# antarcticrainforest/seabreeze_param

Hardware: AMD Instinct MI355X
Metric: grid-points/sec for sea_breeze_diag on N2560x1920 global grid; achieved HBM GB/s (higher is better)
Workload: dtype f64; 1 GPU; seabreeze_diag generic flavour, N1280 (2560x1920) global grid, nz=56, fp64 (BASELINE.json configs[2]); stream=torch's current stream (torch and the library share one HIP runtime), plan_cache=stored, nx=2560, ny=1920, nz=56, search_halo=16, parallelism=latband1, variant=default, comm=none, multi_rank_rccl=unmeasured on hardware so far (one GPU per box in the build pool)

## Files before the change

include/seabreeze_hip.h:

```cpp
#ifndef SEABREEZE_HIP_H
#define SEABREEZE_HIP_H

#include <stddef.h>
#include <stdint.h>

#ifdef __cplusplus
extern "C" {
#endif

typedef struct sb_ctx sb_ctx;

typedef enum sb_status {
    SB_OK = 0,
    SB_ERR_ARG = 1,
    SB_ERR_HIP = 2,
    SB_ERR_NO_DEVICE = 3,
    SB_ERR_ALLOC = 4,
    SB_ERR_COMM = 5
} sb_status;

typedef enum sb_boundary {
    SB_BND_WRAPPER = 0,
    SB_BND_GLOBAL = 1,
    SB_BND_HALO = 2
} sb_boundary;

typedef struct sb_tunables {
    double target_plev_pa;
    double thresh_wind;
    double thresh_winddir;
    double thresh_windch;
    double thresh_thc;
    double target_time_s;
    double maxdist_km;
} sb_tunables;

int  sb_create(sb_ctx **ctx, int device);
int  sb_destroy(sb_ctx *ctx);
const char *sb_last_error(const sb_ctx *ctx);
const char *sb_version(void);
void sb_default_tunables(sb_tunables *t);
int  sb_set_search_radius_hint(sb_ctx *ctx, int radius);
int  sb_set_fold(sb_ctx *ctx, int on);
int  sb_set_plan_cache(sb_ctx *ctx, int on);
int  sb_set_wide_strip(sb_ctx *ctx, int on);
int  sb_set_band_order(sb_ctx *ctx, int contrast_first);
int  sb_set_workgroups(sb_ctx *ctx, int n);
int  sb_set_static_sigma(sb_ctx *ctx, int on);
int  sb_set_table_contrast(sb_ctx *ctx, int on);
int  sb_set_table_window_cache(sb_ctx *ctx, int on);
int  sb_table_cache_report(sb_ctx *ctx, long long rep[4]);
int  sb_last_step_report(sb_ctx *ctx, int report[4]);
int  sb_last_counters(sb_ctx *ctx, long long counters[4]);
int  sb_synchronize(sb_ctx *ctx);
int  sb_profile_begin(sb_ctx *ctx, int max_calls);
int  sb_profile_end(sb_ctx *ctx, double avg_ms[5], int *ncalls);

int sb_seabreeze_diag_f64(sb_ctx *ctx, double timestep_s, int timestep_number,
                          int nx, int ny, int nz, int halo, int bnd,
                          const double *p, const double *u, const double *v,
                          const double *theta, const double *mask, const double *z,
                          const double *sigma, double *windspeed, double *winddir,
                          double *thc, double *sb_con, const sb_tunables *tun);
int sb_seabreeze_diag_f32(sb_ctx *ctx, float timestep_s, int timestep_number,
                          int nx, int ny, int nz, int halo, int bnd,
                          const float *p, const float *u, const float *v,
                          const float *theta, const float *mask, const float *z,
                          const float *sigma, float *windspeed, float *winddir,
                          float *thc, float *sb_con, const sb_tunables *tun);
int sb_seabreeze_diag_f64_dev(sb_ctx *ctx, double timestep_s, int timestep_number,
                          int nx, int ny, int nz, int halo, int bnd,
                          const double *p, const double *u, const double *v,
                          const double *theta, const double *mask, const double *z,
                          const double *sigma, double *windspeed, double *winddir,
                          double *thc, double *sb_con, const sb_tunables *tun,
                          void *stream);
int sb_seabreeze_diag_f32_dev(sb_ctx *ctx, float timestep_s, int timestep_number,
                          int nx, int ny, int nz, int halo, int bnd,
                          const float *p, const float *u, const float *v,
                          const float *theta, const float *mask, const float *z,
                          const float *sigma, float *windspeed, float *winddir,
                          float *thc, float *sb_con, const sb_tunables *tun,
                          void *stream);

#define SB_UM_THETA_TO_T0 1
#define SB_UM_LEVEL_WALK  2
int sb_seabreeze_diag_um_f64(sb_ctx *ctx, double timestep_s, int timestep_number, int nx, int ny, int nz,
                             int halo_s, int halo_l, const double *p, const double *u, const double *v,
                             double *theta, const double *z, const double *sigma, const double *mask,
                             double *windspeed, double *winddir, double *thc, double *sb_con, int flags,
                             int *error);
int sb_seabreeze_diag_um_f32(sb_ctx *ctx, float timestep_s, int timestep_number, int nx, int ny, int nz,
                             int halo_s, int halo_l, const float *p, const float *u, const float *v,
                             float *theta, const float *z, const float *sigma, const float *mask,
                             float *windspeed, float *winddir, float *thc, float *sb_con, int flags,
                             int *error);
int sb_seabreeze_diag_um_f64_dev(sb_ctx *ctx, double timestep_s, int timestep_number, int nx, int ny, int nz,
                             int halo_s, int halo_l, const double *p, const double *u, const double *v,
                             double *theta, const double *z, const double *sigma, const double *mask,
// ... 176 lines not shown
```

seabreeze_param_amd/csrc/sb_capi.hip:

```cpp
#include "../../include/seabreeze_hip.h"
#include "sb_launch.hpp"

#include <dlfcn.h>
#include <rccl/rccl.h>

#include <algorithm>
#include <chrono>
#include <cmath>
#include <condition_variable>
#include <functional>
#include <mutex>
#include <thread>
#include <cstdio>
#include <cstdlib>
#include <cstring>
#include <string>
#include <vector>

namespace {

thread_local std::string g_err;

struct DevBuf {
    void *p = nullptr;
// ... 45 lines not shown
            }
        }
    }
    void loop() {
        unsigned long seen = 0;
        for (;;) {
            {
                std::unique_lock<std::mutex> lk(m_);
                cv_.wait(lk, [&] { return quit_ || epoch_ != seen; });
                if (quit_) return;
                seen = epoch_;
            }
            work();
        }
    }
    std::vector<std::thread> workers_;
    std::mutex m_;
    std::condition_variable cv_, done_cv_;
    const std::function<void(int)> *fn_ = nullptr;
    int next_ = 0, total_ = 0, done_ = 0;
    unsigned long epoch_ = 0;
    bool quit_ = false;
};

enum { SB_TICKET_WORDS = 2 };

struct DiagStream {
    bool active = false;
    HostPool *pool = nullptr;
    int nlons = 0, nlats = 0, esz = 0;
    DevBuf z, sd, cdist, ws, wd, thc, p1, theta, v, u, out;
    void *pin_in[2] = {nullptr, nullptr};
    void *pin_out[2] = {nullptr, nullptr};
    size_t pin_in_cap = 0, pin_out_cap = 0;
    hipEvent_t ev_in[2] = {nullptr, nullptr}, ev_out[2] = {nullptr, nullptr};
    long steps = 0;
    double host_copy_s = 0.0, enqueue_s = 0.0, wait_s = 0.0;
};

struct sb_ctx {
    int device = 0;
    hipStream_t stream = nullptr;
    std::string err;
    int radius_hint = 16;
    int ncu = 256;
    int ncu_dev = 256;
    int static_sigma = 0;
    bool stats_valid = false;
    int host_depth = 0;
    int no_fold = 0;
    int no_plan_cache = 0;
    int no_wide_strip = 0;
    int band_late_wind = 0;
    int table_contrast = 0;
    int table_cache = 0;
    SbTabCache tabc;
    bool tab_rep_reset = true;
    bool tab_last = false;
    long long tab_calls = 0;
    int tab_waves = 0;
    const void *stats_sigma = nullptr;
    int stats_dims[4] = {0, 0, 0, 0};
    int stats_ngathered = 0;
    int rep_launches = 0, rep_rccl = 0, rep_groups = 0, rep_copies = 0;
    DevBuf t0, bandbits, clsbits, tiles, vecs, nws, nwd, coastbits, tile_list, seg_list, stamps, jobcopy, plan;
    DevBuf umbits;
    DevBuf tabA, tabL, tabC, tabS;
    DevBuf tabW, tabRep;
    int plan_key[8] = {0, 0, 0, 0, 0, 0, 0, 0};
    const void *plan_bits = nullptr;
    int call_seq = 0, plan_use = 0;
    bool segs_built = false;
    int tiles_n = 0, tiles_strip = -1, flag_parity = 0;
    int *last_flags = nullptr;
    Moments *partials = nullptr;
    unsigned int *ticket = nullptr;
    void *stats = nullptr;
    int *counters = nullptr;
    int *seg_count = nullptr;
    std::vector<unsigned char> dist_key, dist_hv;
    SbDistTraits dist_traits;
    hipStream_t dist_upload_stream = nullptr;
    std::vector<DevBuf> stage;
    Geo last_g{};
    int last_tiles = 0;
    bool have_last = false;
    const Moments *gathered = nullptr;
    int ngathered = 0;
    std::vector<hipEvent_t> prof_ev;
    std::vector<unsigned> prof_mask;
    int prof_calls = 0, prof_max = 0;
    hipStream_t aux_stream = nullptr;
    hipEvent_t ev_fork = nullptr, ev_join = nullptr, ev_mom = nullptr;
    Moments *band_moments_out = nullptr;
    int band_geo = 0;
    DevBuf band_mom;
    void *rccl_lib = nullptr;
    void *comm = nullptr;
    int rank = 0, nranks = 1;
    DiagStream ds;
};

namespace {

int fail(sb_ctx *c, int code, const std::string &msg) {
    if (c) c->err = msg; else g_err = msg;
// ... 88 lines not shown
    const size_t nseg = (size_t)g.nyh * g.nw;
    const size_t seg_cap = (nseg + SB_SEG_PARTS - 1) / SB_SEG_PARTS;
    if ((rc = ensure(c, c->seg_list, seg_cap * SB_SEG_PARTS * sizeof(SbSegEntry)))) return rc;
    job.tile_list = (int *)c->tile_list.p;
    job.seg_list = (SbSegEntry *)c->seg_list.p;
    job.seg_count = c->seg_count;
    job.seg_cap = (int)seg_cap;
    job.t0_fly = (job.flavour == SB_FLAVOUR_GENERIC) ? 1 : 0;
    if (!job.t0_fly) {
        if ((rc = ensure(c, c->t0, ncell * sizeof(T)))) return rc;
        job.t0 = (T *)c->t0.p;
    }
    if ((rc = ensure(c, c->jobcopy, sizeof(DiagJob<double>)))) return rc;
    job.self = (DiagJob<T> *)c->jobcopy.p;
    const bool cache = c->table_cache != 0 && c->table_contrast != 0 && job.flavour == SB_FLAVOUR_GENERIC &&
                       (g.bnd == BND_GLOBAL || g.bnd == BND_HALO) && g.band == 0 && phases == 3 && c->gathered == nullptr;
    if (strip || cache) {
        const size_t need = 64 + (strip ? (size_t)c->ncu * SB_PLAN_STRIDE : (size_t)0);
        if (c->plan.cap < need) {
            if ((rc = ensure(c, c->plan, need))) return rc;
            HIPCHK(c, hipMemsetAsync(c->plan.p, 0, need, st));
            c->plan_bits = nullptr;
        }
        if (phases & 1) {
            if (c->call_seq == 0x7fffffff) {
                HIPCHK(c, hipMemsetAsync(c->plan.p, 0, need, st));
                c->call_seq = 0;
                c->plan_bits = nullptr;
            }
            ++c->call_seq;
            if (strip) {
                const int key[8] = {g.nx, g.ny, g.h, g.bnd, g.rows, c->ncu, tx, ty | (vb << 24)};
                c->plan_use = c->plan_bits == c->bandbits.p && std::memcmp(key, c->plan_key, sizeof(key)) == 0 ? 1 : 0;
                std::memcpy(c->plan_key, key, sizeof(key));
                c->plan_bits = c->bandbits.p;
            } else c->plan_bits = nullptr;
        }
        job.plan = (char *)c->plan.p + 64;
        job.plan_gen = (int *)c->plan.p;
        job.call_id = c->call_seq;
        job.plan_use = strip && !c->no_plan_cache ? c->plan_use : 0;
    } else if (phases & 1) c->plan_bits = nullptr;
#ifdef SB_STAMPS
    if ((rc = ensure(c, c->stamps, (size_t)4096 * SB_NSTAMP * sizeof(long long)))) return rc;
    job.stamps = (long long *)c->stamps.p;
#endif
    SbLaunchCtx lc{};
    if (phases == 3 && c->prof_calls < c->prof_max) {
        lc.prof_mask = &c->prof_mask[(size_t)c->prof_calls];
        lc.prof = &c->prof_ev[(size_t)SB_PROF_EVENTS * c->prof_calls++];
    }
    lc.stream = st; lc.partials = c->partials; lc.stats = c->stats;
    lc.gathered = c->gathered; lc.ngathered = c->ngathered; lc.ncu = c->ncu;
    lc.moments_out = (phases == 1) ? c->band_moments_out : nullptr;
    lc.moments_event = (phases == 1 && c->nranks > 1) ? c->ev_mom : nullptr;
    lc.stats_ticket = (int *)c->ticket + 1;
    in.phases = phases; in.t0_fly = job.t0_fly != 0; in.moments_out = lc.moments_out != nullptr;
    in.reuse_stats = reuse_stats<T>(c, job.sigma, g.nx, g.ny, g.h);
    in.plan_use = c->plan_use != 0; in.segs_built = c->segs_built;
    in.scan_wgs = sb_scan_workgroups((unsigned)g.nyh * (unsigned)g.nw, c->ncu);
    in.table = c->table_contrast != 0 && job.flavour == SB_FLAVOUR_GENERIC && (g.bnd == BND_GLOBAL || g.bnd == BND_HALO) && g.band == 0;
    const SbDiagPlan plan = sb_plan_diag(in);
    if (plan.table) {
        const size_t nsum = (size_t)((g.nyh + SB_TAB_RB - 1) / SB_TAB_RB) * g.nxh;
        if ((rc = ensure(c, c->tabA, ncell * sizeof(unsigned long long)))) return rc;
        if ((rc = ensure(c, c->tabL, ncell * sizeof(unsigned long long)))) return rc;
        if ((rc = ensure(c, c->tabC, ncell * sizeof(unsigned)))) return rc;
        if ((rc = ensure(c, c->tabS, nsum * (2 * sizeof(unsigned long long) + sizeof(unsigned))))) return rc;
        lc.tables.A = (unsigned long long *)c->tabA.p; lc.tables.L = (unsigned long long *)c->tabL.p; lc.tables.C = (unsigned *)c->tabC.p;
        lc.tables.SA = (unsigned long long *)c->tabS.p; lc.tables.SL = lc.tables.SA + nsum; lc.tables.SC = (unsigned *)(lc.tables.SL + nsum);
    }
    SbTabKey tkey{};
    if (plan.table && cache) {
        if ((rc = ensure(c, c->tabW, (size_t)g.nx * g.ny * sizeof(unsigned)))) return rc;
        if ((rc = ensure(c, c->tabRep, (SB_TAB_REP_HDR + (size_t)2 * SB_TAB_QUERY_WAVES_PER_CU * c->ncu_dev) * sizeof(unsigned)))) return rc;
        tkey = SbTabKey{g.nx, g.ny, g.h, g.bnd, g.rows, c->bandbits.p, c->clsbits.p, c->tabW.p, c->tabC.p};
        lc.tables.W = (unsigned *)c->tabW.p; lc.tables.rep = (unsigned *)c->tabRep.p;
        lc.tables.gen = job.plan_gen; lc.tables.call_id = job.call_id;
        lc.tables.force = sb_tab_cache_decide(c->tabc, tkey, job.call_id) != SB_TAB_STEADY ? 1 : 0;
        lc.tables.rep_reset = c->tab_rep_reset ? 1 : 0;
    }
    if (plan.wind_scratch) {
        if ((rc = ensure(c, c->nws, (size_t)g.nx * g.ny * sizeof(T)))) return rc;
        if ((rc = ensure(c, c->nwd, (size_t)g.nx * g.ny * sizeof(T)))) return rc;
        job.nws = (T *)c->nws.p; job.nwd = (T *)c->nwd.p;
    }
    if (phases == 3) c->rep_launches = c->rep_rccl = c->rep_groups = c->rep_copies = 0;
    {
        const hipError_t le = sb_launch_diag<T>(job, plan, lc);
        if (le != hipSuccess) {
            c->plan_bits = nullptr;
            c->segs_built = false;
            c->stats_valid = false;
            sb_tab_cache_launch_failed(c->tabc);
        }
        if (le == hipErrorInvalidValue) return fail(c, SB_ERR_ARG, "no contrast kernel instance for this halo / tile shape");
        if (le != hipSuccess) return hipfail(c, le, "sb_launch_diag");
    }
    c->rep_launches += plan.nsteps;
    if (lc.tables.W) {
        sb_tab_cache_filled(c->tabc, tkey, job.call_id);
        c->tab_rep_reset = false;
        c->tab_waves = SB_TAB_QUERY_WAVES_PER_CU * c->ncu;
        ++c->tab_calls;
    } else sb_tab_cache_other_call(c->tabc);
    c->tab_last = lc.tables.W != nullptr;
// ... 1264 lines not shown
    if (dptr) HIPCHK(c, hipFree(dptr));
    return SB_OK;
}
int sb_device_upload(sb_ctx *c, void *dst_dev, const void *src_host, size_t nbytes) {
    if (!c) return fail(nullptr, SB_ERR_ARG, "null context");
    if (!dst_dev || !src_host) return fail(c, SB_ERR_ARG, "null pointer");
    HIPCHK(c, hipMemcpyAsync(dst_dev, src_host, nbytes, hipMemcpyHostToDevice, c->stream));
    HIPCHK(c, hipStreamSynchronize(c->stream));
    return SB_OK;
}
int sb_device_download(sb_ctx *c, void *dst_host, const void *src_dev, size_t nbytes) {
    if (!c) return fail(nullptr, SB_ERR_ARG, "null context");
    if (!dst_host || !src_dev) return fail(c, SB_ERR_ARG, "null pointer");
    HIPCHK(c, hipMemcpyAsync(dst_host, src_dev, nbytes, hipMemcpyDeviceToHost, c->stream));
    HIPCHK(c, hipStreamSynchronize(c->stream));
    return SB_OK;
}

int sb_allgather_moments_dev(sb_ctx *c, const double *mine5, double *gathered, void *stream) {
    if (!c) return fail(nullptr, SB_ERR_ARG, "null context");
    if (!mine5 || !gathered) return fail(c, SB_ERR_ARG, "null pointer");
    hipStream_t st = stream ? (hipStream_t)stream : c->stream;
    if (c->nranks == 1) {
        HIPCHK(c, hipMemcpyAsync(gathered, mine5, 5 * sizeof(double), hipMemcpyDeviceToDevice, st));
        c->rep_copies += 1;
        return SB_OK;
    }
    NCCLCHK(c, g_rccl.AllGather(mine5, gathered, 5, ncclDouble, (ncclComm_t)c->comm, st));
    c->rep_rccl += 1;
    return SB_OK;
}

int sb_set_fold(sb_ctx *c, int on) {
    if (!c) return fail(nullptr, SB_ERR_ARG, "null context");
    c->no_fold = on ? 0 : 1;
    return SB_OK;
}

int sb_set_workgroups(sb_ctx *c, int n) {
    if (!c) return fail(nullptr, SB_ERR_ARG, "null context");
    if (n < 0 || n > c->ncu_dev) return fail(c, SB_ERR_ARG, "sb_set_workgroups: 0 (the default) or 1 .. the device's compute units");
    HIPCHK(c, hipDeviceSynchronize());
    c->ncu = n == 0 ? c->ncu_dev : n;
    c->plan_bits = nullptr;
    return SB_OK;
}

int sb_set_band_order(sb_ctx *c, int contrast_first) {
    if (!c) return fail(nullptr, SB_ERR_ARG, "null context");
    c->band_late_wind = contrast_first ? 1 : 0;
    return SB_OK;
}

int sb_set_plan_cache(sb_ctx *c, int on) {
    if (!c) return fail(nullptr, SB_ERR_ARG, "null context");
    c->no_plan_cache = on ? 0 : 1;
    return SB_OK;
}

int sb_set_wide_strip(sb_ctx *c, int on) {
    if (!c) return fail(nullptr, SB_ERR_ARG, "null context");
    c->no_wide_strip = on ? 0 : 1;
    c->plan_bits = nullptr;
    return SB_OK;
}

int sb_set_static_sigma(sb_ctx *c, int on) {
    if (!c) return fail(nullptr, SB_ERR_ARG, "null context");
    c->static_sigma = on ? 1 : 0;
    c->stats_valid = false;
    return SB_OK;
}

int sb_set_table_contrast(sb_ctx *c, int on) {
    if (!c) return fail(nullptr, SB_ERR_ARG, "null context");
    c->table_contrast = on ? 1 : 0;
    return SB_OK;
}

int sb_set_table_window_cache(sb_ctx *c, int on) {
    if (!c) return fail(nullptr, SB_ERR_ARG, "null context");
    c->table_cache = on ? 1 : 0;
    sb_tab_cache_toggled(c->tabc);
    if (on) { c->tab_rep_reset = true; c->tab_calls = 0; }
    return SB_OK;
}

int sb_table_cache_report(sb_ctx *c, long long rep[4]) {
    if (!c) return fail(nullptr, SB_ERR_ARG, "null context");
    if (!rep) return fail(c, SB_ERR_ARG, "null pointer");
    rep[0] = rep[1] = rep[2] = rep[3] = 0;
    if (c->tab_rep_reset || !c->tabRep.p) return SB_OK;
    HIPCHK(c, hipDeviceSynchronize());
    std::vector<unsigned> d(SB_TAB_REP_HDR + (size_t)2 * c->tab_waves);
    HIPCHK(c, hipMemcpy(d.data(), c->tabRep.p, d.size() * sizeof(unsigned), hipMemcpyDeviceToHost));
    if (c->tab_last)
        for (int w = 0; w < c->tab_waves; ++w) { rep[0] += d[SB_TAB_REP_HDR + 2 * w]; rep[1] += d[SB_TAB_REP_HDR + 2 * w + 1]; }
    rep[2] = d[0]; rep[3] = c->tab_calls;
    return SB_OK;
}

int sb_last_step_report(sb_ctx *c, int report[4]) {
    if (!c) return fail(nullptr, SB_ERR_ARG, "null context");
    if (!report) return fail(c, SB_ERR_ARG, "null pointer");
    report[0] = c->rep_launches; report[1] = c->rep_rccl; report[2] = c->rep_groups; report[3] = c->rep_copies;
    return SB_OK;
// ... 5 lines not shown
```

seabreeze_param_amd/csrc/sb_diag_kernels.hip:

```cpp
#include "sb_device.hpp"
#include "sb_launch.hpp"
#include "sb_scan_body.hpp"

#define STATS_NT SB_STATS_NT

__device__ __forceinline__ Moments moments_from_shifted(double c, double s1, double s2, double mn, double mx,
                                                         int cnt) {
    Moments acc = moments_empty();
    if (cnt > 0) {
        acc.n = (double)cnt;
        acc.mean = c + s1 / acc.n;
        acc.m2 = s2 - s1 * s1 / acc.n;
        acc.mn = mn;
        acc.mx = mx;
    }
    return acc;
}

__device__ __forceinline__ void store_partial(Moments acc, Moments *wpart, Moments *__restrict__ partials) {
    acc = block_merge(acc, wpart);
    if (threadIdx.x == 0) partials[blockIdx.x] = acc;
}

template <typename T>
__global__ __launch_bounds__(STATS_NT) void k_stats(const T *__restrict__ ary, int nx, int ny, int ld,
                                                    size_t off0, Moments *__restrict__ partials, int *__restrict__ ticket,
                                                    T *__restrict__ stats, Moments *__restrict__ moments_out) {
    const unsigned n = (unsigned)nx * (unsigned)ny;
    const unsigned stride = gridDim.x * STATS_NT;
    const bool flat = (ld == nx);
    const double c = (double)ary[off0];
    double s1 = 0.0, s2 = 0.0, mn = 1.0e308, mx = -1.0e308;
    int cnt = 0;
    for (unsigned base = blockIdx.x * STATS_NT + threadIdx.x; base < n; base += 8 * stride) {
        double x[8];
#pragma unroll
        for (int q = 0; q < 8; ++q) {
            const unsigned i = base + q * stride;
            x[q] = c;
            if (i < n) {
                const size_t idx = flat ? (size_t)i : (size_t)(i / (unsigned)nx) * ld + (i % (unsigned)nx);
                x[q] = (double)ary[off0 + idx];
            }
        }
#pragma unroll
        for (int q = 0; q < 8; ++q) {
            if (base + q * stride < n) {
                const double d = x[q] - c;
                s1 += d;
                s2 += d * d;
                mn = x[q] < mn ? x[q] : mn;
                mx = x[q] > mx ? x[q] : mx;
// ... 215 lines not shown
            for (int t = t0; t < t1; ++t) cnt += job.tile_nnmax[t] != 0 ? 1 : 0;
            int at = block_excl_scan(cnt, s_w, total);
            for (int t = t0; t < t1; ++t)
                if (job.tile_nnmax[t] != 0) job.tile_list[1 + at++] = t;
        }
        if (tid == 0) job.tile_list[0] = total;
        for (int i = tid; i < job.tile_pad; i += PREP_NT) job.tile_list[1 + total + i] = -1;
        return;
    }
    const int part = (int)blockIdx.x - 2;
    const unsigned nseg = (unsigned)job.g.nyh * (unsigned)job.g.nw;
    const unsigned cap = (unsigned)job.seg_cap;
    const unsigned s0 = min((unsigned)part * cap, nseg), s1 = min(s0 + cap, nseg);
    SbSegEntry *list = job.seg_list + (size_t)part * cap;
    int total;
    if (cap <= (unsigned)(PREP_MAXCH * PREP_NT)) {
        total = block_compact((int)(s1 - s0), s_cnt, s_w, [&](int i) { return job.bandbits[s0 + (unsigned)i] != 0; },
                              [&](int rank, int i) {
                                  SbSegEntry e;
                                  e.word = job.bandbits[s0 + (unsigned)i]; e.seg = s0 + (unsigned)i; e.pad = 0;
                                  list[rank] = e;
                              });
    } else {
        const unsigned per = (cap + PREP_NT - 1) / PREP_NT;
        const unsigned a0 = min(s0 + (unsigned)tid * per, s1), a1 = min(a0 + per, s1);
        int cnt = 0;
        for (unsigned sg = a0; sg < a1; ++sg) cnt += job.bandbits[sg] != 0 ? 1 : 0;
        int at = block_excl_scan(cnt, s_w, total);
        for (unsigned sg = a0; sg < a1; ++sg) {
            const uint64_t w = job.bandbits[sg];
            if (w) { SbSegEntry e; e.word = w; e.seg = sg; e.pad = 0; list[at++] = e; }
        }
    }
    if (tid == 0) job.seg_count[part] = total;
}

#define WIND_NT 256

template <typename T, bool NTL>
__device__ __forceinline__ T sb_ld(const T *p) {
    if constexpr (NTL) return __builtin_nontemporal_load(p);
    else return *p;
}

template <typename T> struct WindCfg { static constexpr int UN = SB_WIND_UN, WGS = SB_WIND_WGS_PER_CU; };
template <> struct WindCfg<float> { static constexpr int UN = SB_WIND_UN_F32, WGS = SB_WIND_WGS_PER_CU_F32; };

#ifdef SB_STAMPS_WIND
#define SB_WT(i) do { if (stl_ && job.stamps) job.stamps[(size_t)gw_ * SB_NSTAMP + (i)] = wall_clock64(); } while (0)
#else
#define SB_WT(i) do { } while (0)
#endif

template <typename T, int UN, int MODE>
__global__ __launch_bounds__(WIND_NT, WindCfg<T>::WGS) void k_wind(DiagJob<T> job) {
    constexpr bool FINAL = MODE != 0;
    const Geo g = job.g;
    const int lane = threadIdx.x & 63;
#ifdef SB_STAMPS_WIND
    const int gw_ = blockIdx.x * (WIND_NT / SB_WAVE) + (threadIdx.x >> 6);
    int nsegs_ = 0;
    bool stl_ = lane == 0;
    if (gw_ < 4096 && lane < SB_NSTAMP && job.stamps) job.stamps[(size_t)gw_ * SB_NSTAMP + lane] = 0;
#endif
    SB_WT(0);
    for (int i = blockIdx.x * WIND_NT + threadIdx.x; i < job.next_flags_n; i += gridDim.x * WIND_NT) job.next_flags[i] = 0;
    const int cnt = lane < SB_SEG_PARTS ? job.seg_count[lane] : 0;
    const int incl = sb_wave_scan_add(cnt);
    const int total = __builtin_amdgcn_readlane(incl, SB_SEG_PARTS - 1);
    const int nwaves = gridDim.x * (WIND_NT / SB_WAVE);
    const int gw = __builtin_amdgcn_readfirstlane(blockIdx.x * (WIND_NT / SB_WAVE) + (threadIdx.x >> 6));
    auto entry = [&](int e) {
        const uint64_t hit = __ballot(lane < SB_SEG_PARTS && e < incl);
        const int part = hit ? __ffsll((unsigned long long)hit) - 1 : 0;
        const int base = __shfl(incl, part) - __shfl(cnt, part);
        return job.seg_list[(size_t)part * job.seg_cap + (e < total ? e - base : 0)];
    };
    const size_t pl = (size_t)g.nx * g.ny;
    const int nz = job.nz;
    int lev1 = 0;
    if (job.flavour != SB_FLAVOUR_GENERIC) {
        T best = fabs(job.p[0] - job.target_plev);
        for (int k = 1; k < nz; ++k) {
            const T a = fabs(job.p[k] - job.target_plev);
            if (a < best) { best = a; lev1 = k; }
        }
    }
    auto segment = [&](const SbSegEntry cur) __attribute__((always_inline)) {
#ifdef SB_STAMPS_WIND
        const int sbase_ = 3 + 4 * (nsegs_ < 6 ? nsegs_ : 6);
        ++nsegs_;
        stl_ = lane == __ffsll((unsigned long long)cur.word) - 1;
        SB_WT(sbase_);
#endif
        const unsigned Y = cur.seg / (unsigned)g.nw, Xw = cur.seg - Y * (unsigned)g.nw;
        const int x = (int)(Xw * 64u) + lane - g.h, y = (int)Y - g.h;
        if (!((cur.word >> lane) & 1ull)) return;
        const size_t o = (size_t)y * g.nx + x;
        T n_thc = T(0), ws_old = T(0), wd_old = T(0);
        if constexpr (FINAL) { n_thc = job.thc[o]; ws_old = job.ws[o]; wd_old = job.wd[o]; }
        int lev = lev1;
        if (job.flavour == SB_FLAVOUR_GENERIC && job.level_rule == 0) {
            const T *pc = job.p + o;
            T best = T(0);
            for (int k0 = 0; k0 < nz; k0 += UN) {
                T d[UN];
#pragma unroll
                for (int q = 0; q < UN; ++q) {
                    const int k = k0 + q < nz ? k0 + q : nz - 1;
                    d[q] = sb_ld<T, true>(pc + (size_t)k * pl);
                }
#pragma unroll
                for (int q = 0; q < UN; ++q) {
                    const int k = k0 + q;
                    const T a = fabs(d[q] - job.target_plev);
                    if (k == 0) best = a;
                    else if (k < nz && a < best) { best = a; lev = k; }
                }
            }
        } else if (job.flavour == SB_FLAVOUR_GENERIC) {
            const T *pc = job.p + o;
            T diff = T(1000000.);
            bool done = false;
            for (int k0 = 0; k0 < nz && !done; k0 += UN) {
                T d[UN];
#pragma unroll
                for (int q = 0; q < UN; ++q) {
                    const int k = k0 + q < nz ? k0 + q : nz - 1;
                    d[q] = sb_ld<T, true>(pc + (size_t)k * pl);
                }
#pragma unroll
                for (int q = 0; q < UN; ++q) {
                    const int k = k0 + q;
                    const T a = fabs(d[q] - job.target_plev);
                    if (!done && k < nz) {
                        if (a <= diff) { lev = k; diff = a; }
                        else done = true;
                    }
                }
            }
        }
#ifdef SB_STAMPS_WIND
        asm volatile("s_waitcnt vmcnt(0)" ::: "memory");
        SB_WT(sbase_ + 1);
#endif
        const T uu = job.u[(size_t)lev * pl + o];
        const T vv = job.v[(size_t)lev * pl + o];
#ifdef SB_STAMPS_WIND
        asm volatile("s_waitcnt vmcnt(0)" ::: "memory");
        SB_WT(sbase_ + 2);
#endif
        const T n_ws = sqrt(uu * uu + vv * vv);
        const T n_wd = atan2(-uu, -vv) * T(57.2957);
        if constexpr (FINAL) {
// ... 15 lines not shown
            if (cur.word) segment(cur);
        }
        return;
    }
    SB_WT(1);
    if (gw >= total) return;
    SbSegEntry ent = entry(gw);
    for (int e = gw; e < total; e += nwaves) {
        const SbSegEntry cur = ent;
        if (e + nwaves < total) ent = entry(e + nwaves);
        segment(cur);
    }
#ifdef SB_STAMPS_WIND
    stl_ = lane == 0;
#endif
    SB_WT(2);
}

template <typename T>
hipError_t sb_launch_stats(const T *ary, int nx, int ny, int ld, size_t off0, Moments *partials, T *stats,
                           Moments *moments_out, int *ticket, hipStream_t st) {
    const size_t n = (size_t)nx * ny;
    int nblk = (int)((n + (size_t)STATS_NT * 8 - 1) / ((size_t)STATS_NT * 8));
    if (nblk < 1) nblk = 1;
    if (nblk > 256) nblk = 256;
    hipLaunchKernelGGL(k_stats<T>, dim3(nblk), dim3(STATS_NT), 0, st, ary, nx, ny, ld, off0, partials, ticket, stats, moments_out);
    return hipGetLastError();
}

template <typename T>
hipError_t sb_launch_sigmoid_apply(const T *ary, T *sm, size_t n, const T *stats, hipStream_t st) {
    int nblk = (int)((n + 255) / 256);
    if (nblk > 4096) nblk = 4096;
    hipLaunchKernelGGL(k_sigmoid_apply<T>, dim3(nblk), dim3(256), 0, st, ary, sm, n, stats);
    return hipGetLastError();
}

#ifndef SB_SCAN_SPT_F32
#define SB_SCAN_SPT_F32 4
#endif
template <typename T> struct SCAN_SPT { static constexpr int value = 2; };
template <> struct SCAN_SPT<float> { static constexpr int value = SB_SCAN_SPT_F32; };

template <typename T>
static void launch_scan(const DiagJob<T> &job, int nblk, Moments *partials, bool stats, hipStream_t st) {
    const bool wr = job.flavour == SB_FLAVOUR_WRAPPER;
    if (wr && stats) hipLaunchKernelGGL((k_scan<T, SCAN_SPT<T>::value, true, true>), dim3(nblk), dim3(STATS_NT), 0, st, job, partials);
    else if (wr) hipLaunchKernelGGL((k_scan<T, SCAN_SPT<T>::value, true, false>), dim3(nblk), dim3(STATS_NT), 0, st, job, partials);
    else if (stats) hipLaunchKernelGGL((k_scan<T, SCAN_SPT<T>::value, false, true>), dim3(nblk), dim3(STATS_NT), 0, st, job, partials);
    else hipLaunchKernelGGL((k_scan<T, SCAN_SPT<T>::value, false, false>), dim3(nblk), dim3(STATS_NT), 0, st, job, partials);
}

template <typename T>
static void launch_wind(const DiagJob<T> &job, int ncu, hipStream_t st) {
    const dim3 wg(ncu * WindCfg<T>::WGS), wb(WIND_NT);
    if (job.wind_final) hipLaunchKernelGGL((k_wind<T, WindCfg<T>::UN, 1>), wg, wb, 0, st, job);
    else hipLaunchKernelGGL((k_wind<T, WindCfg<T>::UN, 0>), wg, wb, 0, st, job);
}

#define SB_EV_BEGIN(k) do { if (ev) { (void)hipEventRecord(ev[2 * (k)], st); *lc.prof_mask |= 1u << (k); } } while (0)
#define SB_EV_END(k)   do { if (ev) (void)hipEventRecord(ev[2 * (k) + 1], st); } while (0)

template <typename T>
static hipError_t launch_contrast(const DiagJob<T> &job, int H, int ncu, hipStream_t st) {
    if (job.strip == 2) return sb_launch_strip32<T>(job, ncu, st);
    return job.strip ? sb_launch_strip<T>(job, ncu, st) : sb_launch_thc<T>(job, H, ncu, st);
}

template <typename T>
hipError_t sb_launch_diag(const DiagJob<T> &job, const SbDiagPlan &plan, const SbLaunchCtx &lc) {
    hipStream_t st = lc.stream;
    hipError_t e = hipSuccess;
    for (int i = 0; i < plan.nsteps; ++i) {
        const SbStep &s = plan.steps[i];
        hipEvent_t *ev = s.prof == SB_PROF_NONE ? nullptr : lc.prof;
        DiagJob<T> j = job;
        j.wind_final = s.wind_final; j.strip_update = s.strip_update; j.lists_stand = s.lists_stand; j.seg_trust = s.seg_trust; j.fold = s.fold;
        if (s.publish) { j.moments_out = lc.moments_out; j.stats_ticket = lc.stats_ticket; }
        if (s.kernel == SB_K_CONTRAST) {
            if (s.stats == SB_STATS_PARTIALS) { j.fold_partials = lc.partials; j.fold_nparts = s.nparts; }
            if (s.stats == SB_STATS_GATHERED) { j.gath = lc.gathered; j.ngath = lc.ngathered; }
            if (s.fold || s.stats == SB_STATS_GATHERED) j.stats_out = (T *)lc.stats;
        }
        const bool ev_open = i == 0 || plan.steps[i - 1].prof != s.prof, ev_close = i + 1 == plan.nsteps || plan.steps[i + 1].prof != s.prof;
        if (ev_open) SB_EV_BEGIN(s.prof);
        switch (s.kernel) {
        case SB_K_SCAN: launch_scan<T>(j, plan.scan_wgs, lc.partials, s.stats == SB_STATS_PARTIALS, st); break;
        case SB_K_PREP:
            hipLaunchKernelGGL(k_prep<T>, dim3(2 + SB_SEG_PARTS), dim3(PREP_NT), 0, st, j, (const Moments *)lc.partials, s.nparts,
                               (T *)lc.stats, (Moments *)nullptr);
            break;
        case SB_K_MERGE: hipLaunchKernelGGL(k_merge_moments<T>, dim3(1), dim3(SB_WAVE), 0, st, lc.gathered, lc.ngathered, (T *)lc.stats); break;
        case SB_K_T0: hipLaunchKernelGGL(k_t0<T>, dim3((j.g.nxh + 255) / 256, j.g.nyh), dim3(256), 0, st, j); break;
        case SB_K_CONTRAST:
            if ((e = s.table ? sb_launch_table_query<T>(j, lc.tables, lc.ncu, st) : launch_contrast<T>(j, plan.contrast.Hk, lc.ncu, st)) != hipSuccess) return e;
            break;
        case SB_K_WIND: launch_wind<T>(j, lc.ncu, st); break;
        case SB_K_TABLE_ROWS: if ((e = sb_launch_table_rows<T>(j, lc.tables, st)) != hipSuccess) return e; break;
        case SB_K_TABLE_COLS: if ((e = sb_launch_table_cols(j.g, lc.tables, st)) != hipSuccess) return e; break;
        }
        if (ev_close) SB_EV_END(s.prof);
        if (s.publish && lc.moments_event && (e = hipEventRecord(lc.moments_event, st)) != hipSuccess) return e;
    }
    return hipGetLastError();
}

template hipError_t sb_launch_stats<float>(const float *, int, int, int, size_t, Moments *, float *, Moments *, int *,
                                           hipStream_t);
template hipError_t sb_launch_stats<double>(const double *, int, int, int, size_t, Moments *, double *, Moments *, int *,
                                            hipStream_t);
template hipError_t sb_launch_sigmoid_apply<float>(const float *, float *, size_t, const float *, hipStream_t);
template hipError_t sb_launch_sigmoid_apply<double>(const double *, double *, size_t, const double *, hipStream_t);
template hipError_t sb_launch_diag<float>(const DiagJob<float> &, const SbDiagPlan &, const SbLaunchCtx &);
template hipError_t sb_launch_diag<double>(const DiagJob<double> &, const SbDiagPlan &, const SbLaunchCtx &);
```

seabreeze_param_amd/csrc/sb_launch.hpp:

```cpp
#pragma once
#include "sb_device.hpp"
#include "sb_diag_plan.hpp"
#include "sb_dist_plan.hpp"

#define SB_STATS_MAX_BLOCKS 2048
#define SB_DIST_TY 4
#define SB_PROF_EVENTS (2 * SB_PROF_KERNELS)
#ifndef SB_WIND_UN
#define SB_WIND_UN 8
#endif
#ifndef SB_WIND_WGS_PER_CU
#define SB_WIND_WGS_PER_CU 4
#endif
#ifndef SB_WIND_UN_F32
#define SB_WIND_UN_F32 14
#endif
#ifndef SB_WIND_WGS_PER_CU_F32
#define SB_WIND_WGS_PER_CU_F32 8
#endif

#define SB_TAB_FB 36
#define SB_TAB_REACH 127
#define SB_TAB_RB 16
static_assert((2 * SB_TAB_REACH + 1) * (2 * SB_TAB_REACH + 1) < (1 << (63 - 11 - SB_TAB_FB)), "a window at the reach must fit 63 bits");
static_assert((2 * SB_TAB_REACH + 3) * (2 * SB_TAB_REACH + 3) >= (1 << (63 - 11 - SB_TAB_FB)), "the reach is the largest the format holds");
#include "sb_table_cache.hpp"
#define SB_TAB_REP_HDR 2
#define SB_TAB_QUERY_WAVES_PER_CU 16
struct SbTables {
    unsigned long long *A, *L, *SA, *SL;
    unsigned *C, *SC;
    unsigned *W;
    unsigned *rep;
    const int *gen;
    int call_id, force, rep_reset;
};
__device__ __forceinline__ bool sb_tab_fill(const SbTables &tb) { return !tb.W || tb.force || *tb.gen == tb.call_id; }

struct SbLaunchCtx {
    hipStream_t stream;
    hipEvent_t *prof;
    unsigned *prof_mask;
    Moments *partials;
    void *stats;
    const Moments *gathered;
    int ngathered;
    Moments *moments_out;
    hipEvent_t moments_event;
    int *stats_ticket;
    int ncu;
    SbTables tables;
};

template <typename T>
hipError_t sb_launch_stats(const T *ary, int nx, int ny, int ld, size_t off0, Moments *partials, T *stats,
                           Moments *moments_out, int *ticket, hipStream_t st);
template <typename T>
hipError_t sb_launch_sigmoid_apply(const T *ary, T *sm, size_t n, const T *stats, hipStream_t st);
inline int sb_scan_workgroups(unsigned nseg, int ncu) {
    const int nblk = (int)((nseg + 31) / 32);
    return nblk < 1 ? 1 : nblk > ncu ? ncu : nblk;
}
template <typename T>
hipError_t sb_launch_diag(const DiagJob<T> &job, const SbDiagPlan &plan, const SbLaunchCtx &lc);
void sb_thc_tile_shape(int H, int *tx, int *ty);
template <typename T>
hipError_t sb_launch_thc(const DiagJob<T> &job, int H, int ncu, hipStream_t st);

template <typename T>
hipError_t sb_launch_strip(const DiagJob<T> &job, int ncu, hipStream_t st);
bool sb_strip_shape(int nx, int rows, int *ntx, int *nty);
template <typename T>
hipError_t sb_launch_strip32(const DiagJob<T> &job, int ncu, hipStream_t st);
template <>
hipError_t sb_launch_strip32<float>(const DiagJob<float> &job, int ncu, hipStream_t st);
template <>
hipError_t sb_launch_strip32<double>(const DiagJob<double> &job, int ncu, hipStream_t st);
bool sb_strip32_shape(int nx, int rows, int *ntx, int *nty);
inline SbShapes sb_contrast_shapes(int nx, int rows) {
    SbShapes s;
    s.strip_fits = sb_strip_shape(nx, rows, &s.strip_ntx, &s.strip_nty);
    s.strip32_fits = sb_strip32_shape(nx, rows, &s.strip32_ntx, &s.strip32_nty);
    sb_thc_tile_shape(24, &s.tile_w, &s.tile_rows24);
    sb_thc_tile_shape(32, &s.tile_w, &s.tile_rows32);
    return s;
}

template <typename T>
hipError_t sb_launch_table_rows(const DiagJob<T> &job, const SbTables &tb, hipStream_t st);
hipError_t sb_launch_table_cols(const Geo &g, const SbTables &tb, hipStream_t st);
template <typename T>
hipError_t sb_launch_table_query(const DiagJob<T> &job, const SbTables &tb, int ncu, hipStream_t st);

template <typename T>
hipError_t sb_launch_theta_to_t0(T *theta, const T *z, const T *sigma, size_t n, const T *stats, hipStream_t st);

template <typename T>
hipError_t sb_launch_edges(const T *lsm, const T *ci, T *coast, int nx, int ny, int rule, int bnd, hipStream_t st);
template <typename T>
hipError_t sb_launch_dist(const T *coast, const T *mask, const T *phi, const T *lamf,
                          const T *shl, const T *chl,
                          T *cdist, int nx, int ny,
                          int k, T maxdist, uint64_t *bits,
// ... 12 lines not shown
```

seabreeze_param_amd/hip.py:

```python
from __future__ import annotations

import ctypes as C
import os

import numpy as np

_HERE = os.path.dirname(os.path.abspath(__file__))
LIB_PATH = os.environ.get("SEABREEZE_HIP_LIB", os.path.join(_HERE, "libseabreeze_hip.so"))

SB_BND_WRAPPER, SB_BND_GLOBAL, SB_BND_HALO = 0, 1, 2
SB_UM_THETA_TO_T0, SB_UM_LEVEL_WALK = 1, 2
SB_DIST_MAX_WINDOW = 255
SB_DIST_UM_MAX_WINDOW = 255

_SFX = {np.dtype(np.float32): "f32", np.dtype(np.float64): "f64"}
_CT = {np.dtype(np.float32): C.c_float, np.dtype(np.float64): C.c_double}


class SeabreezeHipError(RuntimeError):
    pass


class Tunables(C.Structure):
    _fields_ = [(n, C.c_double) for n in (
# ... 47 lines not shown
    return C.c_void_p(int(a))


def _host(a, dt):
    a = np.ascontiguousarray(a, dtype=dt)
    return a


class Context:

    def __init__(self, device: int = -1):
        self.lib = load_library()
        h = C.c_void_p()
        rc = self.lib.sb_create(C.byref(h), C.c_int(device))
        if rc != 0:
            raise SeabreezeHipError(f"sb_create failed ({rc}): {self.lib.sb_last_error(None).decode()}")
        self.h = h

    def close(self):
        if getattr(self, "h", None):
            self.lib.sb_destroy(self.h)
            self.h = None

    def __del__(self):
        try:
            self.close()
        except Exception:
            pass

    def _chk(self, rc, what):
        if rc != 0:
            raise SeabreezeHipError(f"{what} failed ({rc}): {self.lib.sb_last_error(self.h).decode()}")

    def synchronize(self):
        self._chk(self.lib.sb_synchronize(self.h), "sb_synchronize")

    def set_search_radius_hint(self, r: int):
        self._chk(self.lib.sb_set_search_radius_hint(self.h, C.c_int(r)), "sb_set_search_radius_hint")

    def set_fold(self, on: bool):
        self._chk(self.lib.sb_set_fold(self.h, C.c_int(1 if on else 0)), "sb_set_fold")

    def set_plan_cache(self, on: bool):
        self._chk(self.lib.sb_set_plan_cache(self.h, C.c_int(1 if on else 0)), "sb_set_plan_cache")

    def set_wide_strip(self, on: bool):
        self._chk(self.lib.sb_set_wide_strip(self.h, C.c_int(1 if on else 0)), "sb_set_wide_strip")

    def set_workgroups(self, n: int):
        self._chk(self.lib.sb_set_workgroups(self.h, C.c_int(int(n))), "sb_set_workgroups")

    def set_band_order(self, contrast_first: bool):
        self._chk(self.lib.sb_set_band_order(self.h, C.c_int(1 if contrast_first else 0)), "sb_set_band_order")

    def set_static_sigma(self, on: bool):
        self._chk(self.lib.sb_set_static_sigma(self.h, C.c_int(1 if on else 0)), "sb_set_static_sigma")

    def set_table_contrast(self, on: bool):
        self._chk(self.lib.sb_set_table_contrast(self.h, C.c_int(1 if on else 0)), "sb_set_table_contrast")

    def set_table_window_cache(self, on: bool):
        self._chk(self.lib.sb_set_table_window_cache(self.h, C.c_int(1 if on else 0)), "sb_set_table_window_cache")

    def table_cache_report(self):
        arr = (C.c_longlong * 4)()
        self._chk(self.lib.sb_table_cache_report(self.h, arr), "sb_table_cache_report")
        return dict(stored_cells=arr[0], searched_cells=arr[1], fills=arr[2], calls=arr[3])

    def last_step_report(self):
        arr = (C.c_int * 4)()
        self._chk(self.lib.sb_last_step_report(self.h, arr), "sb_last_step_report")
        return dict(kernel_launches=arr[0], rccl_ops=arr[1], rccl_groups=arr[2], d2d_copies=arr[3])

    def last_counters(self):
        arr = (C.c_longlong * 4)()
        self._chk(self.lib.sb_last_counters(self.h, arr), "sb_last_counters")
        return dict(band_cells=arr[0], global_path_cells=arr[1], one_class_cells=arr[2], max_radius=arr[3])

    def profile_begin(self, max_calls: int):
        self._chk(self.lib.sb_profile_begin(self.h, C.c_int(max_calls)), "sb_profile_begin")

    def profile_end(self):
        ms = (C.c_double * 5)()
        n = C.c_int(0)
        self._chk(self.lib.sb_profile_end(self.h, ms, C.byref(n)), "sb_profile_end")
        return dict(k_scan=ms[0], k_wind=ms[1], k_t0=ms[2], k_thc=ms[3], k_prep=ms[4]), n.value

    def seabreeze_diag(self, timestep, tn, p, u, v, theta, mask, z, sigma, ws, wd, thc, sb_con,
                       halo=0, bnd=SB_BND_GLOBAL, tunables: Tunables | None = None):
        dt = np.dtype(ws.dtype)
        sfx, ct = _SFX[dt], _CT[dt]
        p = _host(p, dt); u = _host(u, dt); v = _host(v, dt)
        theta = _host(theta, dt); mask = _host(mask, dt); z = _host(z, dt); sigma = _host(sigma, dt)
        nz, ny, nx = p.shape
        for a in (theta, mask, z, sigma):
            if a.shape != (ny + 2 * halo, nx + 2 * halo):
                raise ValueError(f"2-D input shape {a.shape} != {(ny + 2 * halo, nx + 2 * halo)}")
        for a in (ws, wd, thc, sb_con):
            if a.shape != (ny, nx) or a.dtype != dt or not a.flags.c_contiguous:
                raise ValueError("state arrays must be C-contiguous (ny, nx) of the working dtype")
        fn = getattr(self.lib, f"sb_seabreeze_diag_{sfx}")
        rc = fn(self.h, ct(timestep), C.c_int(tn), C.c_int(nx), C.c_int(ny), C.c_int(nz), C.c_int(halo),
                C.c_int(bnd), _p(p), _p(u), _p(v), _p(theta), _p(mask), _p(z), _p(sigma),
                _p(ws), _p(wd), _p(thc), _p(sb_con), C.byref(tunables) if tunables is not None else None)
        self._chk(rc, "sb_seabreeze_diag")
        return sb_con
# ... 243 lines not shown
```

Before: 42.81 billion grid-points/s.

## Pair adjacent columns in wind level search with 16-byte loads split across half-waves

```diff
diff --git a/include/seabreeze_hip.h b/include/seabreeze_hip.h
--- a/include/seabreeze_hip.h
+++ b/include/seabreeze_hip.h
@@ -45,6 +45,8 @@
 int  sb_set_plan_cache(sb_ctx *ctx, int on);
 int  sb_set_wide_strip(sb_ctx *ctx, int on);
 int  sb_set_band_order(sb_ctx *ctx, int contrast_first);
+int  sb_set_wind_pairs(sb_ctx *ctx, int on);
+int  sb_last_wind_pairs(sb_ctx *ctx, int *ran);
 int  sb_set_workgroups(sb_ctx *ctx, int n);
 int  sb_set_static_sigma(sb_ctx *ctx, int on);
 int  sb_set_table_contrast(sb_ctx *ctx, int on);
diff --git a/seabreeze_param_amd/csrc/sb_capi.hip b/seabreeze_param_amd/csrc/sb_capi.hip
--- a/seabreeze_param_amd/csrc/sb_capi.hip
+++ b/seabreeze_param_amd/csrc/sb_capi.hip
@@ -121,6 +121,8 @@
     int no_plan_cache = 0;
     int no_wide_strip = 0;
     int band_late_wind = 0;
+    int no_wind_pairs = 0;
+    int last_wind_pairs = 0;
     int table_contrast = 0;
     int table_cache = 0;
     SbTabCache tabc;
@@ -315,6 +317,7 @@
     }
     lc.stream = st; lc.partials = c->partials; lc.stats = c->stats;
     lc.gathered = c->gathered; lc.ngathered = c->ngathered; lc.ncu = c->ncu;
+    lc.wind_pairs = c->no_wind_pairs ? 0 : 1; lc.wind_pairs_ran = &c->last_wind_pairs;
     lc.moments_out = (phases == 1) ? c->band_moments_out : nullptr;
     lc.moments_event = (phases == 1 && c->nranks > 1) ? c->ev_mom : nullptr;
     lc.stats_ticket = (int *)c->ticket + 1;
@@ -1685,6 +1688,18 @@
     return SB_OK;
 }
 
+int sb_set_wind_pairs(sb_ctx *c, int on) {
+    if (!c) return fail(nullptr, SB_ERR_ARG, "null context");
+    c->no_wind_pairs = on ? 0 : 1;
+    return SB_OK;
+}
+
+int sb_last_wind_pairs(sb_ctx *c, int *ran) {
+    if (!c || !ran) return fail(c, SB_ERR_ARG, "sb_last_wind_pairs: null argument");
+    *ran = c->last_wind_pairs;
+    return SB_OK;
+}
+
 int sb_set_plan_cache(sb_ctx *c, int on) {
     if (!c) return fail(nullptr, SB_ERR_ARG, "null context");
     c->no_plan_cache = on ? 0 : 1;
diff --git a/seabreeze_param_amd/csrc/sb_diag_kernels.hip b/seabreeze_param_amd/csrc/sb_diag_kernels.hip
--- a/seabreeze_param_amd/csrc/sb_diag_kernels.hip
+++ b/seabreeze_param_amd/csrc/sb_diag_kernels.hip
@@ -1,3 +1,4 @@
+#include <climits>
 #include "sb_device.hpp"
 #include "sb_launch.hpp"
 #include "sb_scan_body.hpp"
@@ -319,7 +320,7 @@
 #define SB_WT(i) do { } while (0)
 #endif
 
-template <typename T, int UN, int MODE>
+template <typename T, int UN, int MODE, bool PAIR = false>
 __global__ __launch_bounds__(WIND_NT, WindCfg<T>::WGS) void k_wind(DiagJob<T> job) {
     constexpr bool FINAL = MODE != 0;
     const Geo g = job.g;
@@ -362,11 +363,55 @@
 #endif
         const unsigned Y = cur.seg / (unsigned)g.nw, Xw = cur.seg - Y * (unsigned)g.nw;
         const int x = (int)(Xw * 64u) + lane - g.h, y = (int)Y - g.h;
-        if (!((cur.word >> lane) & 1ull)) return;
+        if constexpr (!PAIR) {
+            if (!((cur.word >> lane) & 1ull)) return;
+        }
+        const bool mine = PAIR ? ((cur.word >> lane) & 1ull) != 0 : true;
         const size_t o = (size_t)y * g.nx + x;
         T n_thc = T(0), ws_old = T(0), wd_old = T(0);
-        if constexpr (FINAL) { n_thc = job.thc[o]; ws_old = job.ws[o]; wd_old = job.wd[o]; }
+        if constexpr (FINAL) {
+            if (mine) { n_thc = job.thc[o]; ws_old = job.ws[o]; wd_old = job.wd[o]; }
+        }
         int lev = lev1;
+        if constexpr (PAIR) {
+            typedef T pair_t __attribute__((ext_vector_type(2)));
+            constexpr int UNP = SB_WIND_UN_PAIR;
+            const int m = lane & 31, h = lane >> 5;
+            const uint64_t pairmask = (cur.word | cur.word >> 1) & 0x5555555555555555ull;
+            T best0 = T(INFINITY), best1 = T(INFINITY);
+            int lev0 = h ? INT_MAX : 0, lev1p = lev0;
+            if ((pairmask >> (2 * m)) & 1ull) {
+                const T *pc = job.p + ((size_t)y * g.nx + (size_t)((int)(Xw * 64u) + 2 * m - g.h));
+                const int ni = (nz + 1) >> 1;
+                for (int i0 = 0; i0 < ni; i0 += UNP) {
+                    pair_t d[UNP];
+#pragma unroll
+                    for (int q = 0; q < UNP; ++q) {
+                        const int k = 2 * (i0 + q) + h;
+                        d[q] = __builtin_nontemporal_load((const pair_t *)(pc + (size_t)(k < nz ? k : nz - 1) * pl));
+                    }
+#pragma unroll
+                    for (int q = 0; q < UNP; ++q) {
+                        const int k = 2 * (i0 + q) + h;
+                        const T a0 = fabs(d[q].x - job.target_plev), a1 = fabs(d[q].y - job.target_plev);
+                        if (k == 0) { best0 = a0; best1 = a1; }
+                        else if (k < nz) {
+                            if (a0 < best0) { best0 = a0; lev0 = k; }
+                            if (a1 < best1) { best1 = a1; lev1p = k; }
+                        }
+                    }
+                }
+            }
+            {
+                const T o0 = __shfl_xor(best0, 32), o1 = __shfl_xor(best1, 32);
+                const int p0 = __shfl_xor(lev0, 32), p1 = __shfl_xor(lev1p, 32);
+                if (o0 < best0 || (!(best0 < o0) && p0 < lev0)) lev0 = p0;
+                if (o1 < best1 || (!(best1 < o1) && p1 < lev1p)) lev1p = p1;
+            }
+            const int le = __shfl(lev0, lane >> 1), lo = __shfl(lev1p, lane >> 1);
+            if (!mine) return;
+            lev = (lane & 1) ? lo : le;
+        } else
         if (job.flavour == SB_FLAVOUR_GENERIC && job.level_rule == 0) {
             const T *pc = job.p + o;
             T best = T(0);
@@ -488,8 +533,17 @@
 }
 
 template <typename T>
-static void launch_wind(const DiagJob<T> &job, int ncu, hipStream_t st) {
+static void launch_wind(const DiagJob<T> &job, const SbLaunchCtx &lc, hipStream_t st) {
+    const int ncu = lc.ncu;
     const dim3 wg(ncu * WindCfg<T>::WGS), wb(WIND_NT);
+    bool pairs = false;
+    if constexpr (sizeof(T) == 8)
+        pairs = lc.wind_pairs && job.wind_final && job.flavour == SB_FLAVOUR_GENERIC && job.level_rule == 0 &&
+                job.g.nx % 2 == 0 && job.g.h % 2 == 0 && ((uintptr_t)job.p & 15u) == 0;
+    if (lc.wind_pairs_ran) *lc.wind_pairs_ran = pairs ? 1 : 0;
+    if constexpr (sizeof(T) == 8) {
+        if (pairs) { hipLaunchKernelGGL((k_wind<T, WindCfg<T>::UN, 1, true>), wg, wb, 0, st, job); return; }
+    }
     if (job.wind_final) hipLaunchKernelGGL((k_wind<T, WindCfg<T>::UN, 1>), wg, wb, 0, st, job);
     else hipLaunchKernelGGL((k_wind<T, WindCfg<T>::UN, 0>), wg, wb, 0, st, job);
 }
@@ -531,7 +585,7 @@
         case SB_K_CONTRAST:
             if ((e = s.table ? sb_launch_table_query<T>(j, lc.tables, lc.ncu, st) : launch_contrast<T>(j, plan.contrast.Hk, lc.ncu, st)) != hipSuccess) return e;
             break;
-        case SB_K_WIND: launch_wind<T>(j, lc.ncu, st); break;
+        case SB_K_WIND: launch_wind<T>(j, lc, st); break;
         case SB_K_TABLE_ROWS: if ((e = sb_launch_table_rows<T>(j, lc.tables, st)) != hipSuccess) return e; break;
         case SB_K_TABLE_COLS: if ((e = sb_launch_table_cols(j.g, lc.tables, st)) != hipSuccess) return e; break;
         }
diff --git a/seabreeze_param_amd/csrc/sb_launch.hpp b/seabreeze_param_amd/csrc/sb_launch.hpp
--- a/seabreeze_param_amd/csrc/sb_launch.hpp
+++ b/seabreeze_param_amd/csrc/sb_launch.hpp
@@ -17,6 +17,9 @@
 #endif
 #ifndef SB_WIND_WGS_PER_CU_F32
 #define SB_WIND_WGS_PER_CU_F32 8
+#endif
+#ifndef SB_WIND_UN_PAIR
+#define SB_WIND_UN_PAIR 7
 #endif
 
 #define SB_TAB_FB 36
@@ -49,6 +52,8 @@
     hipEvent_t moments_event;
     int *stats_ticket;
     int ncu;
+    int wind_pairs;
+    int *wind_pairs_ran;
     SbTables tables;
 };
 
diff --git a/seabreeze_param_amd/hip.py b/seabreeze_param_amd/hip.py
--- a/seabreeze_param_amd/hip.py
+++ b/seabreeze_param_amd/hip.py
@@ -123,6 +123,14 @@
 
     def set_band_order(self, contrast_first: bool):
         self._chk(self.lib.sb_set_band_order(self.h, C.c_int(1 if contrast_first else 0)), "sb_set_band_order")
+
+    def set_wind_pairs(self, on: bool):
+        self._chk(self.lib.sb_set_wind_pairs(self.h, C.c_int(1 if on else 0)), "sb_set_wind_pairs")
+
+    def last_wind_pairs(self) -> int:
+        ran = C.c_int(0)
+        self._chk(self.lib.sb_last_wind_pairs(self.h, C.byref(ran)), "sb_last_wind_pairs")
+        return ran.value
 
     def set_static_sigma(self, on: bool):
         self._chk(self.lib.sb_set_static_sigma(self.h, C.c_int(1 if on else 0)), "sb_set_static_sigma")
```

Result: faster. 47.64 billion grid-points/s, median of 6 (+11.3%).
